# samuel-watson/glmmrMCML

Hardware: AMD Instinct MI355X
Metric: MCML iters/sec x m chains (simlik evals/sec) (higher is better)
Workload: dtype f64

## Files before the change

### glmmrmcml_amd/api.py

```python
import ctypes as C

import numpy as np

from . import _lib

c_dp = C.POINTER(C.c_double)
c_ip = C.POINTER(C.c_int32)

REDUCE_FN = C.CFUNCTYPE(C.c_int, C.c_void_p, C.c_void_p, C.c_int)


class Problem(C.Structure):
    _fields_ = [("cov", c_ip), ("cov_rows", C.c_int), ("data", c_dp), ("data_len", C.c_int),
                ("eff_range", c_dp), ("eff_len", C.c_int), ("Z", c_dp), ("X", c_dp), ("y", c_dp),
                ("n", C.c_int), ("Q", C.c_int), ("P", C.c_int), ("family", C.c_char_p),
                ("link", C.c_char_p)]


class DevOpts(C.Structure):
    _fields_ = [("device", C.c_int), ("stream", C.c_void_p), ("rank", C.c_int), ("world", C.c_int),
                ("reduce", REDUCE_FN), ("reduce_user", C.c_void_p)]


class HmcOpts(C.Structure):
# ... 258 lines not shown
    def last_kernels(self):
        names = {-1: None, 0: "skinny", 1: "band", 2: "dlds", 3: "reg", 4: "sparse"}
        f = C.c_int(); b = C.c_int()
        _lib.check(_lib.lib().glmmr_mcml_ctx_last_kernels(self._h, C.byref(f), C.byref(b)))
        return names[f.value], names[b.value]

    def band_plan(self, chains, which="fwd"):
        out = (C.c_int * 10)()
        _lib.check(_lib.lib().glmmr_mcml_dbg_band_plan(self._h, {"fwd": 0, "bwd": 1}[which], int(chains), out))
        keys = ("used", "nbands", "tiles", "gn", "nwg", "nred", "nslots", "paired", "nempty", "built")
        d = dict(zip(keys, list(out)))
        for k in ("used", "paired", "built"):
            d[k] = bool(d[k])
        return d

    def sparse_plan(self, chains):
        out = (C.c_longlong * 12)()
        _lib.check(_lib.lib().glmmr_mcml_dbg_sparse_plan(self._h, int(chains), out))
        keys = ("active", "factored", "W", "nnz", "nnz_z", "nnz_l", "nblk", "max_blk", "long_rows", "fused", "qrows", "ncb")
        d = dict(zip(keys, (int(v) for v in out)))
        for k in ("active", "factored", "long_rows"):
            d[k] = bool(d[k])
        return d

    def mcml_optim(self, start, trace=0, mcnr=False, maxfun=0, theta_batch=0):
        start = _f(start).ravel(); R = self.npar()
        b = np.zeros(self.P); t = np.zeros(R); sg = C.c_double()
        e = self._ext(0, 1, maxfun, theta_batch)
        _lib.check(_lib.lib().glmmr_mcml_ctx_optim(self._h, _p(start), start.size, int(trace), int(mcnr),
                                                   C.byref(e), _p(b), _p(t), C.byref(sg)))
# ... 256 lines not shown
```

### glmmrmcml_amd/csrc/band_plan.h

```cpp
#pragma once
#include "common.h"
#include <algorithm>
#include <map>
#include <memory>

namespace mcml {

constexpr int BD_BM = 80, BD_BN = 128, BD_BK = 32, BD_STAGES = 3;
constexpr int BD_A_BYTES = BD_BK * BD_BM * 8;
constexpr int BD_B_BYTES = BD_BK * BD_BN * 8;
constexpr int BD_STAGE_BYTES = BD_A_BYTES + BD_B_BYTES;
constexpr size_t BD_LDS_BYTES = (size_t)BD_STAGES * BD_STAGE_BYTES;
constexpr int BD_NA = 3, BD_NB = 4, BD_PER_TILE = BD_NA + BD_NB;
constexpr int BD_TILE_ELEMS = BD_BM * BD_BN;

struct BandItem { int band, kt0, kt1, slot; };
struct BandRed { int band, s0, s1, pad; };

struct BandPlanDev {
    int gn = 0, nwg = 0, nred = 0, nslots = 0;
    int paired = 0;
    DevBuf items, wg_ptr, red, part;
};

struct SkinnyPlan {
    int nrb = 0, nkc = 0, ldp = 0;
    DevBuf range;
    DevBuf part;
};

struct BandPlan {
    int M = 0, K = 0, nbands = 0;
    std::vector<int> kr;
    long tiles = 0;
    std::map<int, std::unique_ptr<BandPlanDev>> by_gn;
    std::unique_ptr<SkinnyPlan> skinny;

    void reset(int M_, int K_, const std::vector<int>& kr_)
    {
        M = M_; K = K_; kr = kr_; nbands = (M + BD_BM - 1) / BD_BM;
        tiles = 0;
        for (int b = 0; b < nbands; ++b) tiles += kr[2 * b + 1] - kr[2 * b];
        by_gn.clear();
        skinny.reset();
    }

    static bool decompose(const std::vector<int>& kr, int nbands, int gn, int target_wg, std::vector<BandItem>& items,
                          std::vector<int>& wg_ptr, std::vector<BandRed>& red, int& nslots)
    {
        items.clear(); wg_ptr.clear(); red.clear(); nslots = 0;
        const int npairs = (nbands + 1) / 2;
        if ((long)npairs * gn * 5 >= (long)target_wg * 4) {
            for (int p = 0; p < npairs; ++p) {
                wg_ptr.push_back((int)items.size());
                items.push_back({p, kr[2 * p], kr[2 * p + 1], -1});
                const int q = nbands - 1 - p;
                if (q > p) items.push_back({q, kr[2 * q], kr[2 * q + 1], -1});
// ... 32 lines not shown
            const long mid = (lo + hi) / 2;
            if (fill(mid, false) <= nwg) hi = mid; else lo = mid + 1;
        }
        fill(lo, true);
        return false;
    }

    int device_plan(int gn, hipStream_t s, BandPlanDev** out)
    {
        auto it = by_gn.find(gn);
        if (it != by_gn.end()) { *out = it->second.get(); return MCML_OK; }
        std::unique_ptr<BandPlanDev> d(new BandPlanDev());
        std::vector<BandItem> items; std::vector<int> wg_ptr; std::vector<BandRed> red; int nslots = 0;
        d->paired = decompose(kr, nbands, gn, 256, items, wg_ptr, red, nslots) ? 1 : 0;
        d->gn = gn; d->nwg = (int)wg_ptr.size() - 1; d->nred = (int)red.size(); d->nslots = nslots;
        MCML_TRY(d->items.ensure(sizeof(BandItem) * (items.size() + 1)));
        MCML_TRY(d->wg_ptr.ensure(sizeof(int) * wg_ptr.size()));
        MCML_HIP(hipMemcpyAsync(d->items.p, items.data(), sizeof(BandItem) * items.size(), hipMemcpyHostToDevice, s));
        MCML_HIP(hipMemcpyAsync(d->wg_ptr.p, wg_ptr.data(), sizeof(int) * wg_ptr.size(), hipMemcpyHostToDevice, s));
        if (nslots > 0) {
            MCML_TRY(d->red.ensure(sizeof(BandRed) * red.size()));
            MCML_HIP(hipMemcpyAsync(d->red.p, red.data(), sizeof(BandRed) * red.size(), hipMemcpyHostToDevice, s));
            MCML_TRY(d->part.ensure(sizeof(double) * (size_t)nslots * gn * BD_TILE_ELEMS));
        }
        MCML_HIP(hipStreamSynchronize(s));
        *out = d.get();
        by_gn[gn] = std::move(d);
        return MCML_OK;
    }
};

// ... 2 lines not shown
```

### glmmrmcml_amd/csrc/cabi.hip

```cpp
#include "../../include/glmmr_mcml_c.h"
#include "ctx.h"
#include <random>
#include "sparse_plan.h"

using namespace mcml;


namespace mcml {
int hmc_sample(Ctx& c, const double* beta, double var_par, const glmmr_mcml_hmc_opts* o, uint64_t seed,
               uint32_t iter_idx, const double* inj_init, const double* inj_mom, uint8_t* flags_out,
               double* probs_out, glmmr_mcml_hmc_diag* diag, int* ncols_out);
int nuts_sample(Ctx& c, const double* beta, double var_par, const glmmr_mcml_nuts_opts* o, uint64_t seed, uint32_t iter_idx,
                int* depth_out, int* nleap_out, double* eps_out, double* accept_out, glmmr_mcml_nuts_diag* diag,
                int* ncols_out);
}

static int flink_of(const char* family, const char* link)
{
    static const char* tab[12][2] = {
        {"poisson", "log"}, {"poisson", "identity"}, {"binomial", "logit"},
        {"binomial", "log"}, {"binomial", "identity"}, {"binomial", "probit"},
        {"gaussian", "identity"}, {"gaussian", "log"}, {"gamma", "log"},
        {"gamma", "inverse"}, {"gamma", "identity"}, {"beta", "logit"}};
    for (int i = 0; i < 12; i++)
// ... 157 lines not shown
    int nempty = 0;
    for (int b = 0; b < bp.nbands; ++b) nempty += bp.kr[2 * b] == bp.kr[2 * b + 1];
    int nwg = 0, nred = 0, nslots = 0, paired = 0, built = 0;
    auto it = bp.by_gn.find(gn);
    if (it != bp.by_gn.end()) {
        const BandPlanDev& d = *it->second;
        nwg = d.nwg; nred = d.nred; nslots = d.nslots; paired = d.paired; built = 1;
    } else if (bp.nbands > 0) {
        std::vector<BandItem> items; std::vector<int> wg_ptr; std::vector<BandRed> red;
        paired = BandPlan::decompose(bp.kr, bp.nbands, gn, 256, items, wg_ptr, red, nslots) ? 1 : 0;
        nwg = (int)wg_ptr.size() - 1; nred = (int)red.size();
    }
    const int v[10] = {(which ? c.band_bwd : c.band_fwd) ? 1 : 0, bp.nbands, (int)bp.tiles, gn, nwg, nred, nslots,
                       paired, nempty, built};
    for (int i = 0; i < 10; ++i) out10[i] = v[i];
    return MCML_OK;
}

extern "C" int glmmr_mcml_dbg_sparse_plan(glmmr_mcml_ctx* h, int chains, long long* out12)
{
    MCML_REQUIRE(h && chains >= 1 && out12, "dbg_sparse_plan: bad argument");
    const Ctx& c = h->c;
    const SparseZL& sp = c.sp;
    for (int i = 0; i < 12; ++i) out12[i] = 0;
    out12[0] = sp.active ? 1 : 0;
    out12[10] = cm_qrows(c.Q); out12[11] = cm_chain_blocks(chains);
    if (!sp.active) return MCML_OK;
    out12[1] = sp.factored ? 1 : 0; out12[2] = sp.W; out12[3] = sp.nnz; out12[4] = sp.nnz_z; out12[5] = sp.nnz_l;
    out12[6] = sp.nblk; out12[7] = sp.max_blk; out12[8] = cm_long_rows(c) ? 1 : 0; out12[9] = cm_fuse_width(c);
    return MCML_OK;
// ... 212 lines not shown
    if (chains <= 1) return m + 1;
    return chains * ((m + chains - 1) / chains);
}

extern "C" int glmmr_mcml_ctx_profile(glmmr_mcml_ctx* h, int enable, int reset, double* out8)
{
    MCML_REQUIRE(h, "profile: null context");
    Ctx& c = h->c;
    KernelProf& p = c.prof;
    if (out8) {
        out8[0] = p.ms[0]; out8[1] = (double)p.cnt[0]; out8[2] = p.ms[1]; out8[3] = (double)p.cnt[1];
        const double C = (double)c.hmc.C, dense = 2.0 * c.n * (double)c.Q * C;
        double ff = dense, fb = dense, kind = 0;
        if (c.sp.active) { ff = fb = 2.0 * (double)c.sp.nnz * C; kind = 2; }
        else {
            if (c.band_fwd) { ff = 2.0 * 80.0 * 32.0 * (double)c.band_fwd_tiles * C; kind = 1; }
            if (c.band_bwd) { fb = 2.0 * 80.0 * 32.0 * (double)c.band_bwd_tiles * C; kind = 1; }
        }
        out8[4] = ff; out8[5] = fb; out8[6] = dense; out8[7] = kind;
    }
    if (reset) for (int i = 0; i < 4; ++i) { p.ms[i] = 0; p.cnt[i] = 0; p.seen[i] = 0; }
    if (enable && !p.on) {
        MCML_HIP(hipSetDevice(c.device));
        while (p.ev.size() < 4096) { hipEvent_t e; if (hipEventCreate(&e) != hipSuccess) { (void)hipGetLastError(); break; } p.ev.push_back(e); }
    }
    p.on = enable != 0;
    return MCML_OK;
}

extern "C" int glmmr_mcml_ctx_profile_launches(glmmr_mcml_ctx* h, long long* fwd, long long* bwd)
{
    MCML_REQUIRE(h, "profile_launches: null context");
// ... 304 lines not shown
```

### glmmrmcml_amd/csrc/debug_hooks.hip

```cpp
#include "dgemm_mfma.h"
#include "dgemm_dl.h"
#include "dgemm_band.h"

using namespace mcml;

extern "C" int glmmr_mcml_dbg_dgemm(int M, int N, int K, const double* A, int lda,
                                    const double* B, int ldb, int b_nmajor,
                                    double alpha, double beta, double* C, int ldc,
                                    int lower_only, int force_tile)
{
    int ndev = 0;
    if (hipGetDeviceCount(&ndev) != hipSuccess || ndev == 0) {
        set_error("no HIP device: libglmmr_mcml_hip has no CPU fallback");
        return MCML_ENODEVICE;
    }
    hipStream_t s = nullptr;
    DevMat dA, dB, dC;
    if (force_tile == 40) {
        MCML_REQUIRE(!b_nmajor && !lower_only, "dbg_dgemm: the direct-to-LDS kernel takes a K-major B and all tiles");
        const int kpad = round_up(K, 32);
        MCML_TRY(dA.alloc(M, K, 32));
        MCML_HIP(hipMemset(dA.d(), 0, sizeof(double) * (size_t)dA.ld * dA.cols_alloc));
        MCML_HIP(hipMemcpy2D(dA.d(), sizeof(double) * dA.ld, A, sizeof(double) * lda, sizeof(double) * M, K, hipMemcpyHostToDevice));
        MCML_TRY(dB.alloc(kpad, N));
// ... 63 lines not shown
    hipEvent_t e0, e1;
    MCML_HIP(hipEventCreate(&e0));
    MCML_HIP(hipEventCreate(&e1));
    MCML_HIP(hipEventRecord(e0, s));
    for (int i = 0; i < iters; i++) MCML_TRY(go());
    MCML_HIP(hipEventRecord(e1, s));
    MCML_HIP(hipEventSynchronize(e1));
    float ms = 0;
    MCML_HIP(hipEventElapsedTime(&ms, e0, e1));
    *ms_per_launch = ms / iters;
    (void)hipEventDestroy(e0);
    (void)hipEventDestroy(e1);
    return MCML_OK;
}

extern "C" int glmmr_mcml_dbg_dgemm_band(int M, int N, int K, const double* A, int lda, const double* B, int ldb,
                                         double* C, int ldc, int* tiles_executed)
{
    int ndev = 0;
    if (hipGetDeviceCount(&ndev) != hipSuccess || ndev == 0) {
        set_error("no HIP device: libglmmr_mcml_hip has no CPU fallback");
        return MCML_ENODEVICE;
    }
    MCML_REQUIRE(M > 0 && N > 0 && K > 0 && A && B && C, "dbg_dgemm_band: bad argument");
    hipStream_t s = nullptr;
    DevMat dA, dB, dC;
    MCML_TRY(dA.alloc(M, K, 32));
    MCML_HIP(hipMemset(dA.d(), 0, sizeof(double) * (size_t)dA.ld * dA.cols_alloc));
    MCML_HIP(hipMemcpy2D(dA.d(), sizeof(double) * dA.ld, A, sizeof(double) * lda, sizeof(double) * M, K, hipMemcpyHostToDevice));
    MCML_TRY(dB.alloc(round_up(K, 32), N));
    MCML_HIP(hipMemset(dB.d(), 0, sizeof(double) * (size_t)dB.ld * N));
    MCML_HIP(hipMemcpy2D(dB.d(), sizeof(double) * dB.ld, B, sizeof(double) * ldb, sizeof(double) * K, N, hipMemcpyHostToDevice));
    MCML_TRY(dC.alloc(M, N));
    MCML_HIP(hipMemset(dC.d(), 0, sizeof(double) * (size_t)dC.ld * N));
    MCML_REQUIRE(dlds_applicable(M, N, K, dA.d(), dA.ld, dA.cols_alloc, dB.d(), dB.ld), "dbg_dgemm_band: contract");
    const int nbands = (M + BD_BM - 1) / BD_BM;
    DevBuf kr;
    MCML_TRY(kr.ensure(sizeof(int) * 2 * nbands));
    hipLaunchKernelGGL(k_band_ranges, dim3(nbands), dim3(256), 0, s, dA.d(), dA.ld, M, K, kr.as<int>());
    MCML_HIP(hipGetLastError());
    std::vector<int> hk(2 * nbands);
    MCML_HIP(hipMemcpy(hk.data(), kr.p, sizeof(int) * 2 * nbands, hipMemcpyDeviceToHost));
    BandPlan plan;
    plan.reset(M, K, hk);
    if (tiles_executed) *tiles_executed = (int)plan.tiles;
    EpiAxpby epi{dC.d(), dC.ld, 1.0, 0.0};
    MCML_TRY(launch_gemm_band(s, plan, N, dA.d(), dA.ld, dB.d(), dB.ld, epi));
    MCML_TRY(download_matrix(C, ldc, dC.d(), dC.ld, M, N, s));
    return MCML_OK;
}

extern "C" int glmmr_mcml_dbg_band_clocks(int M, int N, int iters, int mode, double* out3)
{
    int ndev = 0;
    if (hipGetDeviceCount(&ndev) != hipSuccess || ndev == 0) {
        set_error("no HIP device: libglmmr_mcml_hip has no CPU fallback");
        return MCML_ENODEVICE;
    }
    hipStream_t s = nullptr;
    if (getenv("GLMMR_MCML_DBG_STREAM")) MCML_HIP(hipStreamCreateWithFlags(&s, hipStreamNonBlocking));
    std::vector<double> hA((size_t)M * M, 0.0), hB((size_t)M * N);
    uint64_t x = 88172645463325252ULL;
    auto rnd = [&]() { x ^= x << 13; x ^= x >> 7; x ^= x << 17; return (double)(x >> 11) / 9007199254740992.0 * 2 - 1; };
    const bool cst = getenv("GLMMR_MCML_DBG_DATA") && !strcmp(getenv("GLMMR_MCML_DBG_DATA"), "const");
    const bool dec = getenv("GLMMR_MCML_DBG_DATA") && !strcmp(getenv("GLMMR_MCML_DBG_DATA"), "decay");
    for (int j = 0; j < M; ++j) for (int i = j; i < M; ++i) hA[i + (size_t)j * M] = cst ? 1.0 : dec ? rnd() * std::exp(-(double)(i - j) / 40.0) : rnd();
    for (auto& v : hB) v = cst ? 1.0 : rnd();
    DevMat dA, dB, dC;
    MCML_TRY(dA.alloc(M, M, 32));
    MCML_HIP(hipMemset(dA.d(), 0, sizeof(double) * (size_t)dA.ld * dA.cols_alloc));
    MCML_HIP(hipMemcpy2D(dA.d(), sizeof(double) * dA.ld, hA.data(), sizeof(double) * M, sizeof(double) * M, M, hipMemcpyHostToDevice));
    MCML_TRY(dB.alloc(round_up(M, 32), N));
    MCML_HIP(hipMemset(dB.d(), 0, sizeof(double) * (size_t)dB.ld * N));
    MCML_HIP(hipMemcpy2D(dB.d(), sizeof(double) * dB.ld, hB.data(), sizeof(double) * M, sizeof(double) * M, N, hipMemcpyHostToDevice));
    MCML_TRY(dC.alloc(M, N));
    const int nbands = (M + BD_BM - 1) / BD_BM;
    DevBuf kr, clk;
    MCML_TRY(kr.ensure(sizeof(int) * 2 * nbands));
    MCML_TRY(clk.ensure(16));
    MCML_HIP(hipMemset(clk.p, 0, 16));
    hipLaunchKernelGGL(k_band_ranges, dim3(nbands), dim3(256), 0, s, dA.d(), dA.ld, M, M, kr.as<int>());
    std::vector<int> hk(2 * nbands);
    MCML_HIP(hipMemcpy(hk.data(), kr.p, sizeof(int) * 2 * nbands, hipMemcpyDeviceToHost));
    BandPlan plan;
    plan.reset(M, M, hk);
    const double tiles = (double)plan.tiles;
    EpiAxpby epi{dC.d(), dC.ld, 1.0, 0.0};
    if (mode < 0) {
        for (int i = 0; i < 3; i++)
            MCML_TRY((launch_gemm_band<EpiAxpby, false>(s, plan, N, dA.d(), dA.ld, dB.d(), dB.ld, epi)));
        hipEvent_t f0, f1;
        MCML_HIP(hipEventCreate(&f0));
        MCML_HIP(hipEventCreate(&f1));
        MCML_HIP(hipEventRecord(f0, s));
        for (int i = 0; i < iters; i++)
            MCML_TRY((launch_gemm_band<EpiAxpby, false>(s, plan, N, dA.d(), dA.ld, dB.d(), dB.ld, epi)));
        MCML_HIP(hipEventRecord(f1, s));
        MCML_HIP(hipEventSynchronize(f1));
        float fms = 0;
        MCML_HIP(hipEventElapsedTime(&fms, f0, f1));
        out3[0] = fms / iters; out3[1] = 0;
// ... 184 lines not shown
```

### glmmrmcml_amd/csrc/dgemm_band.h

```cpp
#pragma once
#include "dgemm_dlds.h"
#include "band_plan.h"

namespace mcml {

struct BandP {
    GemmP g;
    const BandItem* items;
    const int* wg_ptr;
    int nwg;
    double* part;
    int mode;
    unsigned long long* clocks;
};

static __global__ __launch_bounds__(256) void k_band_ranges(const double* A, int lda, int M, int K, int* krange)
{
    __shared__ int smin[256], smax[256];
    const int band = blockIdx.x, r0 = band * BD_BM;
    const int rows = (M - r0 < BD_BM) ? (M - r0) : BD_BM;
    int kmin = 1 << 30, kmax = -1;
    for (int k = threadIdx.x; k < K; k += 256) {
        const double* col = A + r0 + (size_t)k * lda;
        bool nz = false;
        for (int r = 0; r < rows; ++r) nz |= (col[r] != 0.0);
        if (nz) { kmin = min(kmin, k); kmax = max(kmax, k); }
    }
    smin[threadIdx.x] = kmin; smax[threadIdx.x] = kmax;
    __syncthreads();
    for (int o = 128; o > 0; o >>= 1) {
        if ((int)threadIdx.x < o) {
            smin[threadIdx.x] = min(smin[threadIdx.x], smin[threadIdx.x + o]);
            smax[threadIdx.x] = max(smax[threadIdx.x], smax[threadIdx.x + o]);
        }
        __syncthreads();
    }
    if (threadIdx.x == 0) {
        if (smax[0] < 0) { krange[2 * band] = 0; krange[2 * band + 1] = 0; }
        else { krange[2 * band] = smin[0] / BD_BK; krange[2 * band + 1] = smax[0] / BD_BK + 1; }
    }
}

#if defined(__HIP_DEVICE_COMPILE__)
#define BD_RD(dst, addr, off) asm volatile("ds_read_b64 %0, %1 offset:%2" : "=v"(dst) : "v"(addr), "i"(off))
#else
#define BD_RD(dst, addr, off) (dst = 0.0)
#endif
template <int KS>
__device__ __forceinline__ void bd_read(double (&a)[5], double& b, unsigned aaddr, unsigned baddr)
{
    BD_RD(a[0], aaddr, KS * 4 * BD_BM * 8);
    BD_RD(a[1], aaddr, KS * 4 * BD_BM * 8 + 128);
    BD_RD(a[2], aaddr, KS * 4 * BD_BM * 8 + 256);
    BD_RD(a[3], aaddr, KS * 4 * BD_BM * 8 + 384);
// ... 2 lines not shown
}
template <int LEAVE>
__device__ __forceinline__ void bd_wait(double (&a)[5], double& b)
{
#if defined(__HIP_DEVICE_COMPILE__)
    if constexpr (LEAVE == 6)
        asm volatile("s_waitcnt lgkmcnt(6)" : "+v"(a[0]), "+v"(a[1]), "+v"(a[2]), "+v"(a[3]), "+v"(a[4]), "+v"(b));
    else
        asm volatile("s_waitcnt lgkmcnt(0)" : "+v"(a[0]), "+v"(a[1]), "+v"(a[2]), "+v"(a[3]), "+v"(a[4]), "+v"(b));
#endif
}
__device__ __forceinline__ void bd_mfma(d4 (&acc)[5][1], const double (&a)[5], double b)
{
#pragma unroll
    for (int i = 0; i < 5; ++i) acc[i][0] = __builtin_amdgcn_mfma_f64_16x16x4f64(b, a[i], acc[i][0], 0, 0, 0);
}

template <class Epi, bool DBG>
__global__ __launch_bounds__(512) void dgemm_band_kernel(BandP bp, Epi epi)
{
    const GemmP& p = bp.g;
    extern __shared__ __attribute__((aligned(16))) double smem[];
    char* lds = reinterpret_cast<char*>(smem);
    const int tid = threadIdx.x, lane = tid & 63, wave = __builtin_amdgcn_readfirstlane(tid >> 6);
    const int l15 = lane & 15, lk = lane >> 4;
    unsigned long long t0c = 0, t0r = 0;
    if constexpr (DBG)
        if (bp.clocks && blockIdx.x == 0 && tid == 0) { t0c = __builtin_amdgcn_s_memtime(); t0r = __builtin_amdgcn_s_memrealtime(); }

    const int nblk = bp.nwg * p.gn;
// ... 5 lines not shown

    unsigned vob[BD_NB]; int lb[BD_NB];
#pragma unroll
    for (int s = 0; s < BD_NB; ++s) {
        const int c = wave + 8 * s;
        const int kp = c >> 1, n = ((c & 1) << 6) + lane;
        int gn = n0 + n;
        if (gn >= p.N) gn = 0;
        vob[s] = (unsigned)((2 * kp + (size_t)gn * p.ldb) * 8);
        lb[s] = BD_A_BYTES + c * 1024;
    }
    const size_t stepA = (size_t)BD_BK * p.lda * 8;

    const int it0 = bp.wg_ptr[pw], it1 = bp.wg_ptr[pw + 1];
    BandItem item{0, 0, 0, -1};
    int m0 = 0;
    unsigned voa[BD_NA]; int la[BD_NA];
#pragma unroll
    for (int s = 0; s < BD_NA; ++s) {
        int c = wave + 8 * s;
        if (c >= 20) c = wave + 8;
        la[s] = c * 1024;
    }
    const char* sA = nullptr; const char* sB = nullptr;
    auto load_item = [&](int it) {
#if defined(__HIP_DEVICE_COMPILE__)
        {
            typedef int i4s __attribute__((ext_vector_type(4)));
            i4s raw;
            const BandItem* ip = bp.items + it;
            asm volatile("s_load_dwordx4 %0, %1, 0x0\n\ts_waitcnt lgkmcnt(0)" : "=&s"(raw) : "s"(ip) : "memory");
            item.band = raw.x; item.kt0 = raw.y; item.kt1 = raw.z; item.slot = raw.w;
        }
#else
        item = bp.items[it];
#endif
        m0 = item.band * BD_BM;
#pragma unroll
        for (int s = 0; s < BD_NA; ++s) {
            int c = wave + 8 * s;
            if (c >= 20) c = wave + 8;
            const int o = c * 1024 + lane * 16;
            const int k = o / (BD_BM * 8), m = (o - k * BD_BM * 8) >> 3;
            int gm = m0 + m;
            if (gm >= p.M) gm = 0;
            voa[s] = (unsigned)((gm + (size_t)k * p.lda) * 8);
        }
        sA = reinterpret_cast<const char*>(p.A) + (size_t)item.kt0 * stepA;
        sB = reinterpret_cast<const char*>(p.B) + (size_t)item.kt0 * (BD_BK * 8);
    };
    auto issue = [&](int stage) {
// ... 37 lines not shown
        d4 acc[5][1];
#pragma unroll
        for (int i = 0; i < 5; ++i) acc[i][0] = d4{0.0, 0.0, 0.0, 0.0};

        if (nk > 0 && mode == 0) {
            const unsigned lds0 = (unsigned)(size_t)(lds_ptr_t)lds;
            const unsigned aoff = lds0 + lk * (BD_BM * 8) + l15 * 8;
            const unsigned boff = lds0 + BD_A_BYTES + (((lk >> 1) * BD_BN + wave * 16 + l15) << 4) + ((lk & 1) << 3);
            if (!pre) { issued = 0; for (; issued < BD_STAGES - 1 && issued < nk; ++issued) issue(issued); }
            wait_leave(issued - 1);
            __builtin_amdgcn_s_barrier();
            if (first_item) stamp(1);
            int st = 0;
            double ra[2][5], rb[2];
            bd_read<0>(ra[0], rb[0], aoff, boff);
            for (int kt = 0; kt < nk; ++kt) {
                if (issued < nk) {
                    int sn = st + BD_STAGES - 1; if (sn >= BD_STAGES) sn -= BD_STAGES;
                    issue(sn);
                    ++issued;
                }
                const unsigned aaddr = aoff + st * BD_STAGE_BYTES, baddr = boff + st * BD_STAGE_BYTES;
                int stn = st + 1; if (stn >= BD_STAGES) stn = 0;
#define BD_STEP(KS, CUR, NXT)                                   \
                bd_read<KS + 1>(ra[NXT], rb[NXT], aaddr, baddr); \
                bd_wait<6>(ra[CUR], rb[CUR]);                    \
                bd_mfma(acc, ra[CUR], rb[CUR]);                  \
                __builtin_amdgcn_sched_barrier(0);
                BD_STEP(0, 0, 1) BD_STEP(1, 1, 0) BD_STEP(2, 0, 1) BD_STEP(3, 1, 0)
                BD_STEP(4, 0, 1) BD_STEP(5, 1, 0) BD_STEP(6, 0, 1)
#undef BD_STEP
                wait_leave(issued - kt - 2);
                bd_wait<0>(ra[1], rb[1]);
                __builtin_amdgcn_s_barrier();
                if (kt + 1 < nk) bd_read<0>(ra[0], rb[0], aoff + stn * BD_STAGE_BYTES, boff + stn * BD_STAGE_BYTES);
                bd_mfma(acc, ra[1], rb[1]);
                __builtin_amdgcn_sched_barrier(0);
                st = stn;
            }
        } else if (DBG && nk > 0 && mode == 8) {
            int issued = 0;
            for (; issued < BD_STAGES - 1 && issued < nk; ++issued) issue(issued);
            wait_leave(issued - 1);
            __builtin_amdgcn_s_barrier();
            int st = 0;
            for (int kt = 0; kt < nk; ++kt) {
                if (issued < nk) {
                    int sn = st + BD_STAGES - 1; if (sn >= BD_STAGES) sn -= BD_STAGES;
                    issue(sn);
                    ++issued;
                }
                const double* as = reinterpret_cast<const double*>(lds + st * BD_STAGE_BYTES);
                const double* bs = reinterpret_cast<const double*>(lds + st * BD_STAGE_BYTES + BD_A_BYTES);
#pragma unroll
// ... 110 lines not shown
}

template <class Epi, bool DBG = false>
static inline int launch_gemm_band(hipStream_t s, BandPlan& plan, int N, const double* A, int lda,
                                   const double* B, int ldb, const Epi& epi,
                                   unsigned long long* clocks = nullptr, int mode = 0)
{
    const int gn = (N + BD_BN - 1) / BD_BN;
    BandPlanDev* d = nullptr;
    MCML_TRY(plan.device_plan(gn, s, &d));
    BandP bp;
    bp.clocks = clocks;
    bp.mode = mode;
    bp.g = GemmP{plan.M, N, plan.K, A, lda, B, ldb, 0, gn, 0};
    bp.items = d->items.as<BandItem>();
    bp.wg_ptr = d->wg_ptr.as<int>();
    bp.nwg = d->nwg;
    bp.part = d->part.d();
    MCML_TRY(ensure_dynamic_lds(reinterpret_cast<const void*>(&dgemm_band_kernel<Epi, DBG>), (int)BD_LDS_BYTES));
    hipLaunchKernelGGL((dgemm_band_kernel<Epi, DBG>), dim3(d->nwg * gn), dim3(512), BD_LDS_BYTES, s, bp, epi);
    if (d->nred > 0)
        hipLaunchKernelGGL((k_band_reduce<Epi>), dim3(d->nred, gn, 4), dim3(128), 0, s, d->red.as<BandRed>(),
                           d->part.d(), gn, plan.M, N, epi);
    MCML_HIP(hipGetLastError());
    return MCML_OK;
}


}
```

### glmmrmcml_amd/csrc/model.hip

```cpp
#include "ctx.h"
#include "dgemm_mfma.h"
#include "dgemm_band.h"
#include "glm.h"
#include "reduce.h"

namespace mcml {

int model_setup(Ctx& c, const double* Z, const double* X, const double* y)
{
    const int n = c.n, Q = c.Q, P = c.P;
    MCML_TRY(upload_matrix(c.Z, Z, n, Q, n, c.stream));
    MCML_TRY(upload_matrix(c.X, X, n, P, n, c.stream));
    MCML_TRY(c.y.ensure(sizeof(double) * (size_t)pad_ld(n)));
    MCML_TRY(c.xb.ensure(sizeof(double) * (size_t)pad_ld(n)));
    MCML_HIP(hipMemsetAsync(c.y.p, 0, sizeof(double) * (size_t)pad_ld(n), c.stream));
    MCML_HIP(hipMemsetAsync(c.xb.p, 0, sizeof(double) * (size_t)pad_ld(n), c.stream));
    std::vector<double> yy(y, y + n);
    if (c.flink == 8)
        for (auto& v : yy) v = log(v);
    MCML_TRY(copy_h2d(c.y.p, yy.data(), sizeof(double) * n, c.stream));
    size_t nnz = 0; int maxrow = 0;
    std::vector<int> cnt(n, 0);
    for (int j = 0; j < Q; ++j)
        for (int i = 0; i < n; ++i)
// ... 234 lines not shown
    }
    if (c.z_width > 0) {
        MCML_TRY(z_times(c, c.L.d(), c.L.ld, c.Q, c.ZL.d(), c.ZL.ld));
    } else {
        EpiAxpby epi{c.ZL.d(), c.ZL.ld, 1.0, 0.0};
        MCML_TRY(launch_gemm<false>(c.stream, c.n, c.Q, c.Q, c.Z.d(), c.Z.ld, c.L.d(), c.L.ld, epi));
    }
    hipLaunchKernelGGL(k_transpose, dim3((c.n + 31) / 32, (c.Q + 31) / 32), dim3(256), 0, c.stream, c.ZL.d(),
                       c.ZL.ld, c.n, c.Q, c.ZLT.d(), c.ZLT.ld);
    MCML_HIP(hipGetLastError());
    c.band_fwd = c.band_bwd = false;
    const char* env = getenv("GLMMR_MCML_GEMM");
    if (!(env && (!strcmp(env, "reg") || !strcmp(env, "dlds")))) {
        auto ranges = [&](const DevMat& A, int M, int K, BandPlan& plan, bool& use, long& ntiles) -> int {
            const int nb = (M + BD_BM - 1) / BD_BM;
            MCML_TRY(c.kr_scratch.ensure(sizeof(int) * 2 * (size_t)nb));
            hipLaunchKernelGGL(k_band_ranges, dim3(nb), dim3(256), 0, c.stream, A.d(), A.ld, M, K, c.kr_scratch.as<int>());
            MCML_HIP(hipGetLastError());
            std::vector<int> h(2 * (size_t)nb);
            MCML_TRY(copy_d2h(h.data(), c.kr_scratch.p, sizeof(int) * h.size(), c.stream));
            MCML_HIP(hipStreamSynchronize(c.stream));
            if (!(plan.M == M && plan.K == K && plan.kr == h))
                plan.reset(M, K, h);
            const long dense = (long)nb * ((K + BD_BK - 1) / BD_BK);
            use = (env && !strcmp(env, "band")) || plan.tiles * 5 <= dense * 4;
            ntiles = plan.tiles;
            return MCML_OK;
        };
        MCML_TRY(ranges(c.ZL, c.n, c.Q, c.plan_fwd, c.band_fwd, c.band_fwd_tiles));
        MCML_TRY(ranges(c.ZLT, c.Q, c.n, c.plan_bwd, c.band_bwd, c.band_bwd_tiles));
    }
    return MCML_OK;
}

template <int FL>
__global__ __launch_bounds__(256) void k_loglik(const double* ZU, int ldz, int n, int ncols, const double* xb,
                                                const double* y, double var_par, int flink_rt, double* partials)
{
// ... 151 lines not shown
```

### include/glmmr_mcml_c.h

```cpp
#ifndef GLMMR_MCML_C_H
#define GLMMR_MCML_C_H
#include <stdint.h>

#ifdef __cplusplus
extern "C" {
#endif

#define GLMMR_MCML_OK            0
#define GLMMR_MCML_EINVAL       -1
#define GLMMR_MCML_EUNSUPPORTED -2
#define GLMMR_MCML_ENOTPD       -3
#define GLMMR_MCML_ESINGULAR    -4
#define GLMMR_MCML_EHIP         -5
#define GLMMR_MCML_ENODEVICE    -6
#define GLMMR_MCML_ENOMEM       -7

const char* glmmr_mcml_last_error(void);


typedef struct glmmr_mcml_problem {
    const int32_t* cov;
    int            cov_rows;
    const double*  data;
    int            data_len;
// ... 99 lines not shown
    int      device;
    int      theta_batch;
} glmmr_mcml_ext;

int glmmr_mcml_gen_u_samples(const double* Z, const double* L, const double* X, const double* y, int n, int Q, int P,
                             const double* beta, const char* family, const char* link, double sigma, int warmup_iter,
                             int m, const glmmr_mcml_nuts_opts* opts, const glmmr_mcml_ext* ext, double* samples,
                             int lds, int* ncols);

int glmmr_mcml_sample_cols(int m, int chains);
int glmmr_mcml_ctx_ncols(glmmr_mcml_ctx* ctx);
int glmmr_mcml_ctx_profile(glmmr_mcml_ctx* ctx, int enable, int reset, double* out8);
int glmmr_mcml_ctx_profile_launches(glmmr_mcml_ctx* ctx, long long* fwd, long long* bwd);
int glmmr_mcml_ctx_last_kernels(glmmr_mcml_ctx* ctx, int* fwd, int* bwd);
int glmmr_mcml_dbg_band_plan(glmmr_mcml_ctx* ctx, int which, int chains, int* out10);
int glmmr_mcml_dbg_sparse_plan(glmmr_mcml_ctx* ctx, int chains, long long* out12);
int glmmr_mcml_dbg_phase_ms(int enable, int reset, double* out8);
int glmmr_mcml_ctx_npar(glmmr_mcml_ctx* ctx);

int glmmr_mcml_ctx_optim(glmmr_mcml_ctx* ctx, const double* start, int nstart, int trace, int mcnr,
                         const glmmr_mcml_ext* ext, double* beta, double* theta, double* sigma);
int glmmr_mcml_ctx_simlik(glmmr_mcml_ctx* ctx, const double* start, int nstart, int trace,
                          const glmmr_mcml_ext* ext, double* beta, double* theta, double* sigma);
int glmmr_mcml_ctx_hess(glmmr_mcml_ctx* ctx, const double* start, int nstart, double tol, int trace,
                        double* H );
int glmmr_mcml_ctx_aic(glmmr_mcml_ctx* ctx, const double* beta_par, int nbeta, const double* cov_par,
                       int ncov, double* out);
int glmmr_mcml_ctx_full(glmmr_mcml_ctx* ctx, const double* start, int nstart, int mcnr, int m, int maxiter,
                        int warmup, double tol, int verbose, double lambda, int trace, int refresh,
                        int maxsteps, double target_accept, const glmmr_mcml_ext* ext, double* beta,
// ... 70 lines not shown
                                const double* upper, double rhobeg, double rhoend, int maxfun, int width,
                                double* x_out, double* f_out, int* nfev_out, int* rounds_out);
typedef int (*glmmr_mcml_batch_objective)(const double* X, int n, int k, double* F, void* user);
int glmmr_mcml_dbg_bobyqa_rounds(glmmr_mcml_batch_objective fb, void* user, int n, const double* x0, const double* lower,
                                 const double* upper, double rhobeg, double rhoend, int maxfun, int width,
                                 double* x_out, double* f_out, int* nfev_out, int* rounds_out);
int glmmr_mcml_dbg_copy_roundtrip(const double* in, long long ld_in, double* out, long long ld_out, long long rows, long long cols);
int glmmr_mcml_dbg_fd_hessian(glmmr_mcml_objective f, void* user, int n, const double* x, double ndeps,
                              int usebounds, const double* lower, const double* upper, double* H);
int glmmr_mcml_dbg_dgemm_bench(int M, int N, int K, int b_nmajor, int iters, int force_tile,
                               double* ms_per_launch);
int glmmr_mcml_dbg_dgemm_bench2(int M, int N, int K, int b_nmajor, int iters, int force_tile, int lower_only,
                                double beta, double* ms_per_launch);
int glmmr_mcml_dbg_dgemm_band(int M, int N, int K, const double* A, int lda, const double* B, int ldb, double* C,
                              int ldc, int* tiles_executed);
int glmmr_mcml_dbg_band_clocks(int M, int N, int iters, int mode, double* out3);

#ifdef __cplusplus
}
#endif
#endif
```

Measured before the change: 1120.

## Skip MFMAs for 16-row subtiles outside their nonzero K range in band GEMM

The band-range kernel now records a nonzero K-tile range for each 16-row subtile of every 80-row band, not just for the band as a whole. The band GEMM kernel uses these per-subtile ranges. Inside the K range where all subtiles are active it runs the full MFMA step. In the head and tail tiles it issues MFMAs only for the active subtiles, which cuts wasted compute on ragged band edges. The cost is extra per-item metadata loads, branching inside the inner loop, and some added code size and register pressure.

```diff
diff --git a/glmmrmcml_amd/api.py b/glmmrmcml_amd/api.py
--- a/glmmrmcml_amd/api.py
+++ b/glmmrmcml_amd/api.py
@@ -296,6 +296,11 @@
             d[k] = bool(d[k])
         return d
 
+    def band_units(self, which="fwd"):
+        out = (C.c_longlong * 2)()
+        _lib.check(_lib.lib().glmmr_mcml_dbg_band_units(self._h, {"fwd": 0, "bwd": 1}[which], out))
+        return int(out[0]), int(out[1])
+
     def sparse_plan(self, chains):
         out = (C.c_longlong * 12)()
         _lib.check(_lib.lib().glmmr_mcml_dbg_sparse_plan(self._h, int(chains), out))
diff --git a/glmmrmcml_amd/csrc/band_plan.h b/glmmrmcml_amd/csrc/band_plan.h
--- a/glmmrmcml_amd/csrc/band_plan.h
+++ b/glmmrmcml_amd/csrc/band_plan.h
@@ -16,11 +16,13 @@
 
 struct BandItem { int band, kt0, kt1, slot; };
 struct BandRed { int band, s0, s1, pad; };
+constexpr int BD_RT = BD_BM / 16;
+struct BandRows { int rt[BD_RT]; int head, tail, pad; };
 
 struct BandPlanDev {
     int gn = 0, nwg = 0, nred = 0, nslots = 0;
     int paired = 0;
-    DevBuf items, wg_ptr, red, part;
+    DevBuf items, rows, wg_ptr, red, part;
 };
 
 struct SkinnyPlan {
@@ -32,15 +34,61 @@
 struct BandPlan {
     int M = 0, K = 0, nbands = 0;
     std::vector<int> kr;
+    std::vector<int> rt;
     long tiles = 0;
+    long units = 0;
     std::map<int, std::unique_ptr<BandPlanDev>> by_gn;
     std::unique_ptr<SkinnyPlan> skinny;
 
-    void reset(int M_, int K_, const std::vector<int>& kr_)
+    static long executed_units(const std::vector<int>& rt)
     {
-        M = M_; K = K_; kr = kr_; nbands = (M + BD_BM - 1) / BD_BM;
+        long u = 0;
+        for (size_t t = 0; t + 1 < rt.size(); t += 2) u += rt[t + 1] - rt[t];
+        return u;
+    }
+
+    static void host_ranges(const double* A, size_t lda, int M, int K, std::vector<int>& kr, std::vector<int>& rt)
+    {
+        const int nb = (M + BD_BM - 1) / BD_BM;
+        std::vector<int> lo((size_t)nb * BD_RT, 1 << 30), hi((size_t)nb * BD_RT, -1);
+        for (int k = 0; k < K; ++k)
+            for (int r = 0; r < M; ++r)
+                if (A[r + (size_t)k * lda] != 0.0) { lo[r / 16] = std::min(lo[r / 16], k); hi[r / 16] = std::max(hi[r / 16], k); }
+        kr.assign(2 * (size_t)nb, 0); rt.assign(2 * (size_t)nb * BD_RT, 0);
+        for (int b = 0; b < nb; ++b) {
+            int bl = 1 << 30, bh = -1;
+            for (int i = 0; i < BD_RT; ++i) {
+                const size_t t = (size_t)b * BD_RT + i;
+                if (hi[t] < 0) continue;
+                rt[2 * t] = lo[t] / BD_BK; rt[2 * t + 1] = hi[t] / BD_BK + 1;
+                bl = std::min(bl, lo[t]); bh = std::max(bh, hi[t]);
+            }
+            if (bh >= 0) { kr[2 * b] = bl / BD_BK; kr[2 * b + 1] = bh / BD_BK + 1; }
+        }
+    }
+
+    static BandRows item_rows(const BandItem& x, const std::vector<int>& rt)
+    {
+        BandRows r{};
+        const int nk = x.kt1 - x.kt0;
+        int head = 0, tail = nk;
+        for (int i = 0; i < BD_RT; ++i) {
+            const size_t t = 2 * ((size_t)x.band * BD_RT + i);
+            const int a = std::min(std::max(rt[t], x.kt0), x.kt1) - x.kt0;
+            const int b = std::min(std::max(rt[t + 1], x.kt0), x.kt1) - x.kt0;
+            r.rt[i] = a | (b << 16);
+            head = std::max(head, a); tail = std::min(tail, b);
+        }
+        r.head = head; r.tail = std::max(head, tail);
+        return r;
+    }
+
+    void reset(int M_, int K_, const std::vector<int>& kr_, const std::vector<int>& rt_)
+    {
+        M = M_; K = K_; kr = kr_; rt = rt_; nbands = (M + BD_BM - 1) / BD_BM;
         tiles = 0;
         for (int b = 0; b < nbands; ++b) tiles += kr[2 * b + 1] - kr[2 * b];
+        units = executed_units(rt);
         by_gn.clear();
         skinny.reset();
     }
@@ -103,7 +151,12 @@
         std::vector<BandItem> items; std::vector<int> wg_ptr; std::vector<BandRed> red; int nslots = 0;
         d->paired = decompose(kr, nbands, gn, 256, items, wg_ptr, red, nslots) ? 1 : 0;
         d->gn = gn; d->nwg = (int)wg_ptr.size() - 1; d->nred = (int)red.size(); d->nslots = nslots;
+        MCML_REQUIRE((K + BD_BK - 1) / BD_BK < (1 << 15), "band plan: K tile indices are packed into 16 bits");
+        std::vector<BandRows> rows(items.size());
+        for (size_t t = 0; t < items.size(); ++t) rows[t] = item_rows(items[t], rt);
         MCML_TRY(d->items.ensure(sizeof(BandItem) * (items.size() + 1)));
+        MCML_TRY(d->rows.ensure(sizeof(BandRows) * (items.size() + 1)));
+        MCML_HIP(hipMemcpyAsync(d->rows.p, rows.data(), sizeof(BandRows) * rows.size(), hipMemcpyHostToDevice, s));
         MCML_TRY(d->wg_ptr.ensure(sizeof(int) * wg_ptr.size()));
         MCML_HIP(hipMemcpyAsync(d->items.p, items.data(), sizeof(BandItem) * items.size(), hipMemcpyHostToDevice, s));
         MCML_HIP(hipMemcpyAsync(d->wg_ptr.p, wg_ptr.data(), sizeof(int) * wg_ptr.size(), hipMemcpyHostToDevice, s));
diff --git a/glmmrmcml_amd/csrc/cabi.hip b/glmmrmcml_amd/csrc/cabi.hip
--- a/glmmrmcml_amd/csrc/cabi.hip
+++ b/glmmrmcml_amd/csrc/cabi.hip
@@ -195,6 +195,25 @@
     const int v[10] = {(which ? c.band_bwd : c.band_fwd) ? 1 : 0, bp.nbands, (int)bp.tiles, gn, nwg, nred, nslots,
                        paired, nempty, built};
     for (int i = 0; i < 10; ++i) out10[i] = v[i];
+    return MCML_OK;
+}
+
+extern "C" int glmmr_mcml_dbg_band_units(glmmr_mcml_ctx* h, int which, long long* out2)
+{
+    MCML_REQUIRE(h && (which == 0 || which == 1) && out2, "dbg_band_units: bad argument");
+    const BandPlan& bp = which ? h->c.plan_bwd : h->c.plan_fwd;
+    out2[0] = (long long)BD_RT * bp.tiles; out2[1] = bp.units;
+    return MCML_OK;
+}
+
+extern "C" int glmmr_mcml_dbg_band_units_host(int M, int K, const double* A, int lda, long long* out2)
+{
+    MCML_REQUIRE(M > 0 && K > 0 && A && lda >= M && out2, "dbg_band_units_host: bad argument");
+    std::vector<int> kr, rt;
+    BandPlan::host_ranges(A, (size_t)lda, M, K, kr, rt);
+    BandPlan bp;
+    bp.reset(M, K, kr, rt);
+    out2[0] = (long long)BD_RT * bp.tiles; out2[1] = bp.units;
     return MCML_OK;
 }
 
@@ -437,8 +456,8 @@
         double ff = dense, fb = dense, kind = 0;
         if (c.sp.active) { ff = fb = 2.0 * (double)c.sp.nnz * C; kind = 2; }
         else {
-            if (c.band_fwd) { ff = 2.0 * 80.0 * 32.0 * (double)c.band_fwd_tiles * C; kind = 1; }
-            if (c.band_bwd) { fb = 2.0 * 80.0 * 32.0 * (double)c.band_bwd_tiles * C; kind = 1; }
+            if (c.band_fwd) { ff = 2.0 * 16.0 * 32.0 * (double)c.plan_fwd.units * C; kind = 1; }
+            if (c.band_bwd) { fb = 2.0 * 16.0 * 32.0 * (double)c.plan_bwd.units * C; kind = 1; }
         }
         out8[4] = ff; out8[5] = fb; out8[6] = dense; out8[7] = kind;
     }
diff --git a/glmmrmcml_amd/csrc/debug_hooks.hip b/glmmrmcml_amd/csrc/debug_hooks.hip
--- a/glmmrmcml_amd/csrc/debug_hooks.hip
+++ b/glmmrmcml_amd/csrc/debug_hooks.hip
@@ -101,8 +101,22 @@
     return MCML_OK;
 }
 
-extern "C" int glmmr_mcml_dbg_dgemm_band(int M, int N, int K, const double* A, int lda, const double* B, int ldb,
-                                         double* C, int ldc, int* tiles_executed)
+static int dbg_band_ranges(hipStream_t s, const DevMat& dA, int M, int K, DevBuf& scratch, BandPlan& plan)
+{
+    const size_t nb = (size_t)((M + BD_BM - 1) / BD_BM);
+    MCML_TRY(scratch.ensure(sizeof(int) * (2 + 2 * BD_RT) * nb));
+    hipLaunchKernelGGL(k_band_ranges, dim3((unsigned)nb), dim3(256), 0, s, dA.d(), dA.ld, M, K, scratch.as<int>(),
+                       scratch.as<int>() + 2 * nb);
+    MCML_HIP(hipGetLastError());
+    MCML_HIP(hipStreamSynchronize(s));
+    std::vector<int> all((2 + 2 * BD_RT) * nb);
+    MCML_HIP(hipMemcpy(all.data(), scratch.p, sizeof(int) * all.size(), hipMemcpyDeviceToHost));
+    plan.reset(M, K, std::vector<int>(all.begin(), all.begin() + 2 * nb), std::vector<int>(all.begin() + 2 * nb, all.end()));
+    return MCML_OK;
+}
+
+static int dbg_dgemm_band(int M, int N, int K, const double* A, int lda, const double* B, int ldb, double* C, int ldc,
+                          int* tiles_executed, bool ignore_rowtiles, long long* units2)
 {
     int ndev = 0;
     if (hipGetDeviceCount(&ndev) != hipSuccess || ndev == 0) {
@@ -123,18 +137,29 @@
     MCML_REQUIRE(dlds_applicable(M, N, K, dA.d(), dA.ld, dA.cols_alloc, dB.d(), dB.ld), "dbg_dgemm_band: contract");
     const int nbands = (M + BD_BM - 1) / BD_BM;
     DevBuf kr;
-    MCML_TRY(kr.ensure(sizeof(int) * 2 * nbands));
-    hipLaunchKernelGGL(k_band_ranges, dim3(nbands), dim3(256), 0, s, dA.d(), dA.ld, M, K, kr.as<int>());
-    MCML_HIP(hipGetLastError());
-    std::vector<int> hk(2 * nbands);
-    MCML_HIP(hipMemcpy(hk.data(), kr.p, sizeof(int) * 2 * nbands, hipMemcpyDeviceToHost));
     BandPlan plan;
-    plan.reset(M, K, hk);
+    MCML_TRY(dbg_band_ranges(s, dA, M, K, kr, plan));
     if (tiles_executed) *tiles_executed = (int)plan.tiles;
+    if (units2) { units2[0] = (long long)BD_RT * plan.tiles; units2[1] = plan.units; }
     EpiAxpby epi{dC.d(), dC.ld, 1.0, 0.0};
-    MCML_TRY(launch_gemm_band(s, plan, N, dA.d(), dA.ld, dB.d(), dB.ld, epi));
+    if (ignore_rowtiles)
+        MCML_TRY((launch_gemm_band<EpiAxpby, true>(s, plan, N, dA.d(), dA.ld, dB.d(), dB.ld, epi, nullptr, 64)));
+    else
+        MCML_TRY(launch_gemm_band(s, plan, N, dA.d(), dA.ld, dB.d(), dB.ld, epi));
     MCML_TRY(download_matrix(C, ldc, dC.d(), dC.ld, M, N, s));
     return MCML_OK;
+}
+
+extern "C" int glmmr_mcml_dbg_dgemm_band(int M, int N, int K, const double* A, int lda, const double* B, int ldb,
+                                         double* C, int ldc, int* tiles_executed)
+{
+    return dbg_dgemm_band(M, N, K, A, lda, B, ldb, C, ldc, tiles_executed, false, nullptr);
+}
+
+extern "C" int glmmr_mcml_dbg_dgemm_band_rowtiles(int M, int N, int K, const double* A, int lda, const double* B,
+                                                  int ldb, double* C, int ldc, int ignore_rowtiles, long long* units2)
+{
+    return dbg_dgemm_band(M, N, K, A, lda, B, ldb, C, ldc, nullptr, ignore_rowtiles != 0, units2);
 }
 
 extern "C" int glmmr_mcml_dbg_band_clocks(int M, int N, int iters, int mode, double* out3)
@@ -163,15 +188,11 @@
     MCML_TRY(dC.alloc(M, N));
     const int nbands = (M + BD_BM - 1) / BD_BM;
     DevBuf kr, clk;
-    MCML_TRY(kr.ensure(sizeof(int) * 2 * nbands));
     MCML_TRY(clk.ensure(16));
     MCML_HIP(hipMemset(clk.p, 0, 16));
-    hipLaunchKernelGGL(k_band_ranges, dim3(nbands), dim3(256), 0, s, dA.d(), dA.ld, M, M, kr.as<int>());
-    std::vector<int> hk(2 * nbands);
-    MCML_HIP(hipMemcpy(hk.data(), kr.p, sizeof(int) * 2 * nbands, hipMemcpyDeviceToHost));
     BandPlan plan;
-    plan.reset(M, M, hk);
-    const double tiles = (double)plan.tiles;
+    MCML_TRY(dbg_band_ranges(s, dA, M, M, kr, plan));
+    const double tiles = (mode >= 0 && (mode & 64)) ? (double)plan.tiles : (double)plan.units / BD_RT;
     EpiAxpby epi{dC.d(), dC.ld, 1.0, 0.0};
     if (mode < 0) {
         for (int i = 0; i < 3; i++)
diff --git a/glmmrmcml_amd/csrc/dgemm_band.h b/glmmrmcml_amd/csrc/dgemm_band.h
--- a/glmmrmcml_amd/csrc/dgemm_band.h
+++ b/glmmrmcml_amd/csrc/dgemm_band.h
@@ -7,6 +7,7 @@
 struct BandP {
     GemmP g;
     const BandItem* items;
+    const BandRows* rows;
     const int* wg_ptr;
     int nwg;
     double* part;
@@ -14,30 +15,39 @@
     unsigned long long* clocks;
 };
 
-static __global__ __launch_bounds__(256) void k_band_ranges(const double* A, int lda, int M, int K, int* krange)
-{
-    __shared__ int smin[256], smax[256];
+static __global__ __launch_bounds__(256) void k_band_ranges(const double* A, int lda, int M, int K, int* krange, int* rtrange)
+{
+    __shared__ int smin[BD_RT], smax[BD_RT];
     const int band = blockIdx.x, r0 = band * BD_BM;
     const int rows = (M - r0 < BD_BM) ? (M - r0) : BD_BM;
-    int kmin = 1 << 30, kmax = -1;
+    if (threadIdx.x < BD_RT) { smin[threadIdx.x] = 1 << 30; smax[threadIdx.x] = -1; }
+    __syncthreads();
+    int kmin[BD_RT], kmax[BD_RT];
+#pragma unroll
+    for (int i = 0; i < BD_RT; ++i) { kmin[i] = 1 << 30; kmax[i] = -1; }
     for (int k = threadIdx.x; k < K; k += 256) {
         const double* col = A + r0 + (size_t)k * lda;
-        bool nz = false;
-        for (int r = 0; r < rows; ++r) nz |= (col[r] != 0.0);
-        if (nz) { kmin = min(kmin, k); kmax = max(kmax, k); }
-    }
-    smin[threadIdx.x] = kmin; smax[threadIdx.x] = kmax;
+#pragma unroll
+        for (int i = 0; i < BD_RT; ++i) {
+            bool nz = false;
+            for (int r = 16 * i; r < 16 * i + 16 && r < rows; ++r) nz |= (col[r] != 0.0);
+            if (nz) { kmin[i] = min(kmin[i], k); kmax[i] = max(kmax[i], k); }
+        }
+    }
+#pragma unroll
+    for (int i = 0; i < BD_RT; ++i)
+        if (kmax[i] >= 0) { atomicMin(&smin[i], kmin[i]); atomicMax(&smax[i], kmax[i]); }
     __syncthreads();
-    for (int o = 128; o > 0; o >>= 1) {
-        if ((int)threadIdx.x < o) {
-            smin[threadIdx.x] = min(smin[threadIdx.x], smin[threadIdx.x + o]);
-            smax[threadIdx.x] = max(smax[threadIdx.x], smax[threadIdx.x + o]);
-        }
-        __syncthreads();
-    }
     if (threadIdx.x == 0) {
-        if (smax[0] < 0) { krange[2 * band] = 0; krange[2 * band + 1] = 0; }
-        else { krange[2 * band] = smin[0] / BD_BK; krange[2 * band + 1] = smax[0] / BD_BK + 1; }
+        int lo = 1 << 30, hi = -1;
+        for (int i = 0; i < BD_RT; ++i) {
+            int* o = rtrange + 2 * (band * BD_RT + i);
+            if (smax[i] < 0) { o[0] = 0; o[1] = 0; continue; }
+            o[0] = smin[i] / BD_BK; o[1] = smax[i] / BD_BK + 1;
+            lo = min(lo, smin[i]); hi = max(hi, smax[i]);
+        }
+        if (hi < 0) { krange[2 * band] = 0; krange[2 * band + 1] = 0; }
+        else { krange[2 * band] = lo / BD_BK; krange[2 * band + 1] = hi / BD_BK + 1; }
     }
 }
 
@@ -70,6 +80,12 @@
 {
 #pragma unroll
     for (int i = 0; i < 5; ++i) acc[i][0] = __builtin_amdgcn_mfma_f64_16x16x4f64(b, a[i], acc[i][0], 0, 0, 0);
+}
+__device__ __forceinline__ void bd_mfma_some(d4 (&acc)[5][1], const double (&a)[5], double b, unsigned act)
+{
+#pragma unroll
+    for (int i = 0; i < 5; ++i)
+        if (act & (1u << i)) acc[i][0] = __builtin_amdgcn_mfma_f64_16x16x4f64(b, a[i], acc[i][0], 0, 0, 0);
 }
 
 template <class Epi, bool DBG>
@@ -105,6 +121,7 @@
 
     const int it0 = bp.wg_ptr[pw], it1 = bp.wg_ptr[pw + 1];
     BandItem item{0, 0, 0, -1};
+    BandRows rows{};
     int m0 = 0;
     unsigned voa[BD_NA]; int la[BD_NA];
 #pragma unroll
@@ -118,14 +135,26 @@
 #if defined(__HIP_DEVICE_COMPILE__)
         {
             typedef int i4s __attribute__((ext_vector_type(4)));
-            i4s raw;
+            typedef int i8s __attribute__((ext_vector_type(8)));
+            i4s raw; i8s rr;
             const BandItem* ip = bp.items + it;
-            asm volatile("s_load_dwordx4 %0, %1, 0x0\n\ts_waitcnt lgkmcnt(0)" : "=&s"(raw) : "s"(ip) : "memory");
+            const BandRows* rp = bp.rows + it;
+            asm volatile("s_load_dwordx4 %0, %2, 0x0\n\ts_load_dwordx8 %1, %3, 0x0\n\ts_waitcnt lgkmcnt(0)"
+                         : "=&s"(raw), "=&s"(rr) : "s"(ip), "s"(rp) : "memory");
             item.band = raw.x; item.kt0 = raw.y; item.kt1 = raw.z; item.slot = raw.w;
+            rows.rt[0] = rr[0]; rows.rt[1] = rr[1]; rows.rt[2] = rr[2]; rows.rt[3] = rr[3]; rows.rt[4] = rr[4];
+            rows.head = rr[5]; rows.tail = rr[6];
         }
 #else
         item = bp.items[it];
+        rows = bp.rows[it];
 #endif
+        if constexpr (DBG)
+            if (bp.mode & 64) {
+                const int nk = item.kt1 - item.kt0;
+                for (int i = 0; i < BD_RT; ++i) rows.rt[i] = nk << 16;
+                rows.head = 0; rows.tail = nk;
+            }
         m0 = item.band * BD_BM;
 #pragma unroll
         for (int s = 0; s < BD_NA; ++s) {
@@ -193,30 +222,51 @@
             int st = 0;
             double ra[2][5], rb[2];
             bd_read<0>(ra[0], rb[0], aoff, boff);
-            for (int kt = 0; kt < nk; ++kt) {
-                if (issued < nk) {
-                    int sn = st + BD_STAGES - 1; if (sn >= BD_STAGES) sn -= BD_STAGES;
-                    issue(sn);
-                    ++issued;
-                }
-                const unsigned aaddr = aoff + st * BD_STAGE_BYTES, baddr = boff + st * BD_STAGE_BYTES;
-                int stn = st + 1; if (stn >= BD_STAGES) stn = 0;
-#define BD_STEP(KS, CUR, NXT)                                   \
+#define BD_MF_ALL(a, b) bd_mfma(acc, a, b)
+#define BD_MF_SOME(a, b) bd_mfma_some(acc, a, b, act)
+#define BD_STEP(MF, KS, CUR, NXT)                                \
                 bd_read<KS + 1>(ra[NXT], rb[NXT], aaddr, baddr); \
                 bd_wait<6>(ra[CUR], rb[CUR]);                    \
-                bd_mfma(acc, ra[CUR], rb[CUR]);                  \
+                MF(ra[CUR], rb[CUR]);                            \
                 __builtin_amdgcn_sched_barrier(0);
-                BD_STEP(0, 0, 1) BD_STEP(1, 1, 0) BD_STEP(2, 0, 1) BD_STEP(3, 1, 0)
-                BD_STEP(4, 0, 1) BD_STEP(5, 1, 0) BD_STEP(6, 0, 1)
+#define BD_KTILE(MF)                                                                                              \
+                if (issued < nk) {                                                                                \
+                    int sn = st + BD_STAGES - 1; if (sn >= BD_STAGES) sn -= BD_STAGES;                            \
+                    issue(sn);                                                                                    \
+                    ++issued;                                                                                     \
+                }                                                                                                 \
+                const unsigned aaddr = aoff + st * BD_STAGE_BYTES, baddr = boff + st * BD_STAGE_BYTES;            \
+                int stn = st + 1; if (stn >= BD_STAGES) stn = 0;                                                  \
+                BD_STEP(MF, 0, 0, 1) BD_STEP(MF, 1, 1, 0) BD_STEP(MF, 2, 0, 1) BD_STEP(MF, 3, 1, 0)               \
+                BD_STEP(MF, 4, 0, 1) BD_STEP(MF, 5, 1, 0) BD_STEP(MF, 6, 0, 1)                                    \
+                           \
+                               \
+                wait_leave(issued - kt - 2);                                                                      \
+                bd_wait<0>(ra[1], rb[1]);                                                                         \
+                __builtin_amdgcn_s_barrier();                                                                     \
+                if (kt + 1 < nk) bd_read<0>(ra[0], rb[0], aoff + stn * BD_STAGE_BYTES, boff + stn * BD_STAGE_BYTES); \
+                MF(ra[1], rb[1]);                                                                                 \
+                __builtin_amdgcn_sched_barrier(0);                                                                \
+                st = stn;
+            const int khead = rows.head, ktail = rows.tail;
+            for (int kt = 0; kt < nk;) {
+                if (kt >= khead && kt < ktail) {
+                    for (; kt < ktail; ++kt) { BD_KTILE(BD_MF_ALL) }
+                } else {
+                    unsigned act = 0;
+#pragma unroll
+                    for (int i = 0; i < BD_RT; ++i) {
+                        const unsigned lo = (unsigned)rows.rt[i] & 0xffffu, hi = (unsigned)rows.rt[i] >> 16;
+                        act |= ((unsigned)kt - lo < hi - lo ? 1u : 0u) << i;
+                    }
+                    BD_KTILE(BD_MF_SOME)
+                    ++kt;
+                }
+            }
+#undef BD_KTILE
 #undef BD_STEP
-                wait_leave(issued - kt - 2);
-                bd_wait<0>(ra[1], rb[1]);
-                __builtin_amdgcn_s_barrier();
-                if (kt + 1 < nk) bd_read<0>(ra[0], rb[0], aoff + stn * BD_STAGE_BYTES, boff + stn * BD_STAGE_BYTES);
-                bd_mfma(acc, ra[1], rb[1]);
-                __builtin_amdgcn_sched_barrier(0);
-                st = stn;
-            }
+#undef BD_MF_SOME
+#undef BD_MF_ALL
         } else if (DBG && nk > 0 && mode == 8) {
             int issued = 0;
             for (; issued < BD_STAGES - 1 && issued < nk; ++issued) issue(issued);
@@ -357,6 +407,7 @@
     bp.mode = mode;
     bp.g = GemmP{plan.M, N, plan.K, A, lda, B, ldb, 0, gn, 0};
     bp.items = d->items.as<BandItem>();
+    bp.rows = d->rows.as<BandRows>();
     bp.wg_ptr = d->wg_ptr.as<int>();
     bp.nwg = d->nwg;
     bp.part = d->part.d();
diff --git a/glmmrmcml_amd/csrc/model.hip b/glmmrmcml_amd/csrc/model.hip
--- a/glmmrmcml_amd/csrc/model.hip
+++ b/glmmrmcml_amd/csrc/model.hip
@@ -272,14 +272,16 @@
     if (!(env && (!strcmp(env, "reg") || !strcmp(env, "dlds")))) {
         auto ranges = [&](const DevMat& A, int M, int K, BandPlan& plan, bool& use, long& ntiles) -> int {
             const int nb = (M + BD_BM - 1) / BD_BM;
-            MCML_TRY(c.kr_scratch.ensure(sizeof(int) * 2 * (size_t)nb));
-            hipLaunchKernelGGL(k_band_ranges, dim3(nb), dim3(256), 0, c.stream, A.d(), A.ld, M, K, c.kr_scratch.as<int>());
+            MCML_TRY(c.kr_scratch.ensure(sizeof(int) * (2 + 2 * BD_RT) * (size_t)nb));
+            hipLaunchKernelGGL(k_band_ranges, dim3(nb), dim3(256), 0, c.stream, A.d(), A.ld, M, K, c.kr_scratch.as<int>(),
+                               c.kr_scratch.as<int>() + 2 * (size_t)nb);
             MCML_HIP(hipGetLastError());
-            std::vector<int> h(2 * (size_t)nb);
-            MCML_TRY(copy_d2h(h.data(), c.kr_scratch.p, sizeof(int) * h.size(), c.stream));
+            std::vector<int> all((2 + 2 * BD_RT) * (size_t)nb);
+            MCML_TRY(copy_d2h(all.data(), c.kr_scratch.p, sizeof(int) * all.size(), c.stream));
             MCML_HIP(hipStreamSynchronize(c.stream));
-            if (!(plan.M == M && plan.K == K && plan.kr == h))
-                plan.reset(M, K, h);
+            const std::vector<int> h(all.begin(), all.begin() + 2 * (size_t)nb), hrt(all.begin() + 2 * (size_t)nb, all.end());
+            if (!(plan.M == M && plan.K == K && plan.kr == h && plan.rt == hrt))
+                plan.reset(M, K, h, hrt);
             const long dense = (long)nb * ((K + BD_BK - 1) / BD_BK);
             use = (env && !strcmp(env, "band")) || plan.tiles * 5 <= dense * 4;
             ntiles = plan.tiles;
diff --git a/include/glmmr_mcml_c.h b/include/glmmr_mcml_c.h
--- a/include/glmmr_mcml_c.h
+++ b/include/glmmr_mcml_c.h
@@ -137,6 +137,8 @@
 int glmmr_mcml_ctx_profile_launches(glmmr_mcml_ctx* ctx, long long* fwd, long long* bwd);
 int glmmr_mcml_ctx_last_kernels(glmmr_mcml_ctx* ctx, int* fwd, int* bwd);
 int glmmr_mcml_dbg_band_plan(glmmr_mcml_ctx* ctx, int which, int chains, int* out10);
+int glmmr_mcml_dbg_band_units(glmmr_mcml_ctx* ctx, int which, long long* out2);
+int glmmr_mcml_dbg_band_units_host(int M, int K, const double* A, int lda, long long* out2);
 int glmmr_mcml_dbg_sparse_plan(glmmr_mcml_ctx* ctx, int chains, long long* out12);
 int glmmr_mcml_dbg_phase_ms(int enable, int reset, double* out8);
 int glmmr_mcml_ctx_npar(glmmr_mcml_ctx* ctx);
@@ -237,6 +239,8 @@
                                 double beta, double* ms_per_launch);
 int glmmr_mcml_dbg_dgemm_band(int M, int N, int K, const double* A, int lda, const double* B, int ldb, double* C,
                               int ldc, int* tiles_executed);
+int glmmr_mcml_dbg_dgemm_band_rowtiles(int M, int N, int K, const double* A, int lda, const double* B, int ldb,
+                                       double* C, int ldc, int ignore_rowtiles, long long* units2);
 int glmmr_mcml_dbg_band_clocks(int M, int N, int iters, int mode, double* out3);
 
 #ifdef __cplusplus
```

Result: slower. 1083 (-3.3%).
